# eldenpark/halo2-pse

Measured on AMD Instinct MI355X. Metric: bn254_msm_g1_adds_per_sec, higher is better.
Workload: dtype u32x8 (256-bit Montgomery integers)

## Files before the change

### halo2-pse_amd/csrc/msm.hip

```cpp
#include <hip/hip_ext.h>
#include <string.h>

#include <atomic>
#include <condition_variable>
#include <thread>
#include <vector>

#include "ecq.h"
#include "engine.h"
#include "host64.h"

namespace h2 {

#define MSM_MAX_C1 1024u
#define MSM_MAX_L 12u
#define MSM_STAGE 16384u
#define MSM_COUNT_TILE 4096u

struct MsmPlan {
    uint32_t c;
    uint32_t W;
    uint32_t q;
    uint32_t cb;
    uint32_t NB;
    uint32_t shared;
    uint32_t heavy_t;
    uint32_t chunk;
};

template <class F>
__device__ __forceinline__ void for_each_digit(const Fe& s, uint32_t c, uint32_t q, uint32_t W, F&& f) {
    uint64_t buf = 0;
    uint32_t nb = 0, w = 0, carry = 0;
    uint32_t width = q ? c : c - 1;
    auto emit = [&]() {
        uint32_t d = ((uint32_t)buf & ((1u << width) - 1)) + carry;
        uint32_t neg = 0;
        carry = 0;
        if (d > (1u << (width - 1))) {
            d = (1u << width) - d;
            neg = 1;
            carry = 1;
        }
        if (d) f(w, d - 1, neg);
        w++;
        buf >>= width;
        nb = nb > width ? nb - width : 0;
        width = w < q ? c : c - 1;
    };
#pragma unroll
    for (int limb = 0; limb < 8; limb++) {
        buf |= (uint64_t)s.l[limb] << nb;
        nb += 32;
        while (nb >= width && w < W) emit();
    }
    while (w < W) emit();
}

struct L1Args {
    const Fe* scalars_one;
    const Fe* const* list;
    uint32_t n, c, q, W, cb, L, C1;
    uint32_t shared, stride;
    uint32_t tile;
    uint16_t* tile_hist;
    const uint32_t* tile_off;
    uint2* tmp;
    uint32_t* tmp_e;
    uint16_t* tmp_k;
    const Affine* chk_bases;
    const Affine* chk_samples;
    uint32_t* chk_flag;
    size_t chk_n, chk_total;
};

__device__ __forceinline__ Fe fr_to_canonical(const Fe& x) {
    Fu c32 = fu_zero();
    c32.l[0] = 32;
    return fu_mul_canon<FrU>(fu_slice(x), c32);
}

#define MSM_TCHUNK 64u
#ifndef MSM_SCATTER_XG
#define MSM_SCATTER_XG 4u
#endif

__global__ void __launch_bounds__(256) msm_l1_count_kernel(L1Args a) {
    __shared__ uint32_t lh[MSM_MAX_C1];
    if (a.chk_flag && blockIdx.x == 0 && blockIdx.y == 0 && threadIdx.x < 4 * H2_PIN_SAMPLES) {
        const uint32_t k = threadIdx.x >> 2, part = threadIdx.x & 3;
// ... 94 lines not shown
        for_each_digit(sc, a.c, a.q, a.W, [&](uint32_t w, uint32_t slot, uint32_t neg) {
            const uint32_t gb = ((set0 + (a.shared ? 0u : w)) << a.cb) | slot;
            const uint32_t pos = atomicAdd(&cur[gb >> a.L], 1u);
            stage[pos] = make_uint2((a.shared ? w * a.stride + i : i) | (neg << 31), gb);
        });
    }
    __syncthreads();
    for (uint32_t pos = threadIdx.x; pos < total; pos += 1024) {
        const uint2 e = stage[pos];
        const uint32_t at = pos + delta[e.y >> a.L];
        if (SPLIT) {
            a.tmp_e[at] = e.x;
            a.tmp_k[at] = (uint16_t)(e.y & ((1u << a.L) - 1));
        } else {
            a.tmp[at] = e;
        }
    }
}

__global__ void __launch_bounds__(1024) msm_l1_scan_kernel(uint32_t* __restrict__ chunk_sum, uint32_t n_chunks, uint32_t C1,
                                                           uint32_t* __restrict__ bin_total, uint32_t* __restrict__ zero, uint32_t zero_words) {
    __shared__ uint32_t part_sum[16][64];
    if (blockIdx.x == 0)
        for (uint32_t i = threadIdx.x; i < zero_words; i += 1024) zero[i] = 0;
    const uint32_t lb = threadIdx.x & 63, p = threadIdx.x >> 6, b = blockIdx.x * 64 + lb;
    const uint32_t per = (n_chunks + 15) / 16, c0 = p * per, c1 = c0 + per < n_chunks ? c0 + per : n_chunks;
    uint32_t sum = 0;
    if (b < C1)
        for (uint32_t ch = c0; ch < c1; ch++) sum += chunk_sum[(size_t)ch * C1 + b];
    part_sum[p][lb] = sum;
    __syncthreads();
    uint32_t acc = 0, all = 0;
#pragma unroll
    for (uint32_t q = 0; q < 16; q++) {
        const uint32_t v = part_sum[q][lb];
        if (q < p) acc += v;
        all += v;
    }
    if (b < C1) {
        for (uint32_t ch = c0; ch < c1; ch++) {
            const uint32_t v = chunk_sum[(size_t)ch * C1 + b];
            chunk_sum[(size_t)ch * C1 + b] = acc;
            acc += v;
        }
        if (p == 0) bin_total[b] = all;
    }
}

__global__ void __launch_bounds__(256) msm_l1_offsets_kernel(const uint16_t* __restrict__ tile_hist, uint32_t n_tiles, uint32_t C1,
                                                             const uint32_t* __restrict__ chunk_sum, const uint32_t* __restrict__ bin_total,
                                                             uint32_t* __restrict__ coarse_start, uint32_t* __restrict__ tile_off) {
    __shared__ uint32_t cs[MSM_MAX_C1], ps[4];
    const uint32_t per = (C1 + 255) / 256;
    uint32_t total;
    uint32_t run = block_scan_base<256>(bin_total, C1, per, ps, &total);
    for (uint32_t j = 0; j < per; j++) {
        const uint32_t k = threadIdx.x * per + j;
        if (k < C1) {
            cs[k] = run;
            run += bin_total[k];
        }
    }
    __syncthreads();
    const uint32_t b = blockIdx.y * 256 + threadIdx.x;
    if (b >= C1) return;
    if (blockIdx.x == 0) {
        coarse_start[b] = cs[b];
        if (b == 0) coarse_start[C1] = total;
    }
    const uint32_t t0 = blockIdx.x * MSM_TCHUNK, t1 = t0 + MSM_TCHUNK < n_tiles ? t0 + MSM_TCHUNK : n_tiles;
    uint32_t running = cs[b] + chunk_sum[(size_t)blockIdx.x * C1 + b];
#pragma unroll 8
    for (uint32_t t = t0; t < t1; t++) {
        tile_off[(size_t)t * C1 + b] = running;
        running += tile_hist[(size_t)t * C1 + b];
    }
}

__device__ __forceinline__ uint32_t size_class(uint32_t cnt, uint32_t bin_shift) {
    uint32_t b = cnt >> bin_shift;
    return 255u - (b < 255u ? b : 255u);
}

template <bool SPLIT>
__global__ void __launch_bounds__(1024) msm_l2_kernel(const uint2* __restrict__ tmp, const uint32_t* __restrict__ tmp_e, const uint16_t* __restrict__ tmp_k,
                                                      const uint32_t* __restrict__ coarse_start, uint32_t L,
                                                      uint32_t bin_shift, uint32_t* __restrict__ vals, uint32_t* __restrict__ start,
                                                      uint32_t* __restrict__ counts, uint32_t* __restrict__ perm, uint32_t* __restrict__ class_hist) {
    constexpr uint32_t NBMAX = 1u << MSM_MAX_L, EPT = MSM_STAGE / 1024;
    __shared__ uint32_t sval[MSM_STAGE];
    __shared__ uint16_t skey[MSM_STAGE];
    __shared__ uint32_t gpos[NBMAX];
    __shared__ uint32_t tcur[NBMAX];
    __shared__ uint32_t tdelta[NBMAX];
    __shared__ uint32_t ps[16], cls[256];
    const uint32_t nb = 1u << L, t = threadIdx.x, per = (nb + 1023) / 1024;
    const uint32_t cs = coarse_start[blockIdx.x], ce = coarse_start[blockIdx.x + 1];
    const bool single = ce - cs <= MSM_STAGE;
    auto load_tile = [&](uint2 (&e)[EPT], uint32_t first, uint32_t tile_n) {
#pragma unroll
        for (uint32_t j = 0; j < EPT; j++) {
            const uint32_t idx = t + j * 1024;
            if (idx < tile_n) e[j] = SPLIT ? make_uint2(tmp_e[first + idx], tmp_k[first + idx]) : tmp[first + idx];
        }
    };
    auto count_tile = [&](const uint2 (&e)[EPT], uint32_t tile_n) {
#pragma unroll
        for (uint32_t j = 0; j < EPT; j++)
            if (t + j * 1024 < tile_n) atomicAdd(&tcur[e[j].y & (nb - 1)], 1u);
    };
    uint2 e[EPT], e_next[EPT];
    const uint32_t first_n = ce - cs < MSM_STAGE ? ce - cs : MSM_STAGE;
    load_tile(e, cs, first_n);
    for (uint32_t k = t; k < nb; k += 1024) tcur[k] = 0;
    if (t < 256) cls[t] = 0;
    __syncthreads();
    if (single) {
        count_tile(e, first_n);
    } else {
        uint32_t idx = cs + t;
        for (; idx + 7 * 1024 < ce; idx += 8 * 1024) {
            uint32_t key[8];
#pragma unroll
            for (uint32_t j = 0; j < 8; j++) key[j] = SPLIT ? (uint32_t)tmp_k[idx + j * 1024] : tmp[idx + j * 1024].y;
#pragma unroll
            for (uint32_t j = 0; j < 8; j++) atomicAdd(&tcur[key[j] & (nb - 1)], 1u);
        }
        for (; idx < ce; idx += 1024) atomicAdd(&tcur[(SPLIT ? (uint32_t)tmp_k[idx] : tmp[idx].y) & (nb - 1)], 1u);
    }
    __syncthreads();
    uint32_t total;
    uint32_t run = block_scan_base<1024>(tcur, nb, per, ps, &total);
    const uint32_t gb0 = blockIdx.x << L;
    for (uint32_t j = 0; j < per; j++) {
        const uint32_t k = t * per + j;
        if (k < nb) {
            const uint32_t cnt = tcur[k];
            gpos[k] = cs + run;
            start[gb0 + k] = cs + run;
            counts[gb0 + k] = cnt;
            atomicAdd(&cls[size_class(cnt, bin_shift)], 1u);
            run += cnt;
        }
    }
    __syncthreads();
    if (class_hist) {
        if (t < 256 && cls[t]) atomicAdd(&class_hist[t], cls[t]);
    } else {
        uint32_t dummy;
        const uint32_t c0 = block_scan_base<1024>(cls, 256, 1, ps, &dummy);
        if (t < 256) tdelta[t] = c0;
        __syncthreads();
        for (uint32_t j = 0; j < per; j++) {
            const uint32_t k = t * per + j;
            if (k < nb) perm[gb0 + atomicAdd(&tdelta[size_class(tcur[k], bin_shift)], 1u)] = gb0 + k;
        }
        __syncthreads();
    }
    for (uint32_t base = cs; base < ce; base += MSM_STAGE) {
        const uint32_t tile_n = ce - base < MSM_STAGE ? ce - base : MSM_STAGE;
        const uint32_t next = base + MSM_STAGE;
        const uint32_t next_n = next < ce ? (ce - next < MSM_STAGE ? ce - next : MSM_STAGE) : 0;
        if (next_n) load_tile(e_next, next, next_n);
        if (!single) {
            for (uint32_t k = t; k < nb; k += 1024) tcur[k] = 0;
            __syncthreads();
            count_tile(e, tile_n);
            __syncthreads();
        }
        run = block_scan_base<1024>(tcur, nb, per, ps, &total);
        for (uint32_t j = 0; j < per; j++) {
            const uint32_t k = t * per + j;
            if (k < nb) {
                const uint32_t cnt = tcur[k];
                tdelta[k] = gpos[k] - run;
                gpos[k] += cnt;
                tcur[k] = run;
                run += cnt;
            }
        }
        __syncthreads();
#pragma unroll
        for (uint32_t j = 0; j < EPT; j++) {
            const uint32_t idx = t + j * 1024;
            if (idx < tile_n) {
                const uint32_t k = e[j].y & (nb - 1);
                const uint32_t pos = atomicAdd(&tcur[k], 1u);
                sval[pos] = e[j].x;
                skey[pos] = (uint16_t)k;
            }
        }
        __syncthreads();
        for (uint32_t pos = t; pos < tile_n; pos += 1024) vals[pos + tdelta[skey[pos]]] = sval[pos];
        __syncthreads();
#pragma unroll
        for (uint32_t j = 0; j < EPT; j++) e[j] = e_next[j];
    }
}

#define MSM_BS_PER 4u
struct HeavyBucket {
    uint32_t bucket, first_chunk, n_chunks, arrived;
};
struct HeavyChunk {
    uint32_t begin, end, owner;
};

__global__ void __launch_bounds__(1024) msm_bucket_scatter_kernel(const uint32_t* __restrict__ counts, const uint32_t* __restrict__ start, uint32_t n_buckets,
                                                                  uint32_t bin_shift, uint32_t heavy_t, uint32_t chunk, uint32_t* __restrict__ hist,
                                                                  uint32_t* __restrict__ perm, uint32_t* __restrict__ heavy_counts,
                                                                  HeavyBucket* __restrict__ heavy_buckets, HeavyChunk* __restrict__ heavy_chunks) {
    __shared__ uint32_t scan[256], lh[256], lbase[256], ps[16];
    const uint32_t t = threadIdx.x;
    for (uint32_t j = 0; j < MSM_BS_PER; j++) {
        const uint32_t b = (blockIdx.x * 1024 + t) * MSM_BS_PER + j;
        const uint32_t cnt = b < n_buckets ? counts[b] : 0;
        if (cnt > heavy_t) {
            const uint32_t s0 = start[b], e0 = s0 + cnt, nch = (cnt + chunk - 1) / chunk;
            const uint32_t slot = atomicAdd(&heavy_counts[1], nch);
            const uint32_t hb = atomicAdd(&heavy_counts[0], 1u);
            const HeavyBucket h = {b, slot, nch, 0};
            heavy_buckets[hb] = h;
            for (uint32_t q = 0; q < nch; q++) {
                const HeavyChunk ch = {s0 + q * chunk, (s0 + (q + 1) * chunk < e0) ? s0 + (q + 1) * chunk : e0, hb};
                heavy_chunks[slot + q] = ch;
            }
        }
    }
    if (!perm) return;
    if (t < 256) lh[t] = 0;
    uint32_t total;
    const uint32_t excl = block_scan_base<1024>(hist, 256, 1, ps, &total);
    if (t < 256) scan[t] = excl;
    __syncthreads();
    uint32_t cls[MSM_BS_PER], rank[MSM_BS_PER];
    const uint32_t b0 = (blockIdx.x * 1024 + t) * MSM_BS_PER;
#pragma unroll
    for (uint32_t j = 0; j < MSM_BS_PER; j++) {
        cls[j] = 0;
        rank[j] = 0;
        if (b0 + j < n_buckets) {
            cls[j] = size_class(counts[b0 + j], bin_shift);
            rank[j] = atomicAdd(&lh[cls[j]], 1u);
        }
    }
    __syncthreads();
    if (t < 256 && lh[t]) lbase[t] = atomicAdd(&hist[256 + t], lh[t]);
    __syncthreads();
#pragma unroll
    for (uint32_t j = 0; j < MSM_BS_PER; j++)
        if (b0 + j < n_buckets) perm[scan[cls[j]] + lbase[cls[j]] + rank[j]] = b0 + j;
}

__device__ __noinline__ void msm_heavy_role(const Affine* __restrict__ bases, const uint32_t* __restrict__ vals, const uint32_t* __restrict__ heavy_counts,
                                            HeavyBucket* __restrict__ heavy_buckets, const HeavyChunk* __restrict__ heavy_chunks,
                                            XYZZu* __restrict__ chunk_sums, uint32_t split_log, uint32_t cont, XYZZu* __restrict__ parts, uint32_t hgrid,
                                            XYZZu* sh);

#ifdef H2_ACCUM_TIMELINE
__device__ unsigned long long g_accum_tl[6 * 16384];
#endif
__global__ void __launch_bounds__(256, 4) msm_accum_kernel(const Affine* __restrict__ bases, const uint32_t* __restrict__ vals,
                                                        const uint32_t* __restrict__ start, const uint32_t* __restrict__ counts,
                                                        const uint32_t* __restrict__ perm, uint32_t n_buckets, uint32_t split_log, uint32_t heavy_t,
                                                        uint32_t cont, XYZZu* __restrict__ parts, uint32_t hgrid, const uint32_t* __restrict__ heavy_counts,
                                                        HeavyBucket* __restrict__ heavy_buckets, const HeavyChunk* __restrict__ heavy_chunks,
                                                        XYZZu* __restrict__ chunk_sums) {
    __shared__ __align__(16) unsigned char lds_raw[256 * sizeof(XYZZu)];
    if (blockIdx.x < hgrid) {
        msm_heavy_role(bases, vals, heavy_counts, heavy_buckets, heavy_chunks, chunk_sums, split_log, cont, parts, hgrid, reinterpret_cast<XYZZu*>(lds_raw));
        return;
    }
    uint32_t t = (blockIdx.x - hgrid) * blockDim.x + threadIdx.x;
    if ((t >> split_log) >= n_buckets) return;
    const uint32_t S = 1u << split_log, sub = t & (S - 1);
    const uint32_t b = perm[t >> split_log];
    uint32_t s = start[b], e = s + counts[b];
#ifdef H2_ACCUM_TIMELINE
    const unsigned long long tl0 = wall_clock64(), tc0 = clock64();
// ... 319 lines not shown
        }
    }
    if (role == 0) sh[quad] = acc;
    __syncthreads();
    for (uint32_t stride = G >> 1; stride >= 1; stride >>= 1) {
        if (g < stride) {
            XYZZu x = sh[quad];
            xyzzu_add_q(x, sh[quad + stride], role);
            if (role == 0) sh[quad] = x;
        }
        __syncthreads();
    }
    if (live && g == 0 && role == 0) J.out[task] = sh[quad];
}

__global__ void __launch_bounds__(64) msm_final_quad_kernel(FinalArgs args, uint32_t n_groups, XYZZu* __restrict__ partials, uint32_t* __restrict__ done,
                                                            XYZZ* __restrict__ set_sums) {
    __shared__ XYZZu sh[16];
    __shared__ uint32_t is_last;
    const uint32_t set = blockIdx.x / n_groups, group = blockIdx.x - set * n_groups;
    const uint32_t quad = threadIdx.x >> 2, role = threadIdx.x & 3;
    uint32_t e = group * 16 + quad;
    const XYZZu* base = nullptr;
    uint32_t stride = 0, o = 0, k = 0, nbits = 0;
    bool found = false;
#pragma unroll
    for (uint32_t i = 0; i < 4; i++) {
        if (i < args.n_arr && !found) {
            if (e < args.arr[i].len) {
                found = true;
                base = args.arr[i].base;
                stride = args.arr[i].stride;
                o = args.arr[i].o;
                k = args.arr[i].k;
                nbits = args.arr[i].nbits;
            } else {
                e -= args.arr[i].len;
            }
        }
    }
    XYZZu x = xyzzu_identity();
    if (found) {
        const uint32_t wgt = (e + o) << k;
        if (wgt) x = xyzzu_mul_small_q(base[(size_t)set * stride + e], wgt, nbits, role);
    }
    if (role == 0) sh[quad] = x;
    __syncthreads();
    for (uint32_t st = 8; st >= 1; st >>= 1) {
        if (quad < st) {
            XYZZu a = sh[quad];
            xyzzu_add_q(a, sh[quad + st], role);
            if (role == 0) sh[quad] = a;
        }
        __syncthreads();
    }
    if (n_groups == 1) {
        if (threadIdx.x == 0) set_sums[set] = xyzzu_to_ext(sh[0]);
        return;
    }
    if (threadIdx.x == 0) {
        partials[blockIdx.x] = sh[0];
        __threadfence();
        is_last = atomicAdd(&done[set], 1u) == n_groups - 1;
    }
    __syncthreads();
    if (!is_last) return;
    __builtin_amdgcn_fence(__ATOMIC_ACQUIRE, "agent");
    x = xyzzu_identity();
    if (quad < n_groups) x = partials[(size_t)set * n_groups + quad];
    if (role == 0) sh[quad] = x;
    __syncthreads();
    for (uint32_t st = 8; st >= 1; st >>= 1) {
        if (quad < st) {
            XYZZu a = sh[quad];
            xyzzu_add_q(a, sh[quad + st], role);
            if (role == 0) sh[quad] = a;
        }
        __syncthreads();
    }
    if (threadIdx.x == 0) set_sums[set] = xyzzu_to_ext(sh[0]);
}

#define MSM_PLANES_MAX 32
#define MSM_PLANE_SETS_MAX 4
struct PlaneJob {
    const XYZZu* base;
    uint32_t log_len;
    uint32_t o;
    uint32_t n_planes;
    uint32_t wgs;
    uint32_t first_plane;
    uint32_t first_block;
};
struct PlaneArgs {
    PlaneJob job[2];
    uint32_t blocks_per_set, planes_per_set;
};

__global__ void __launch_bounds__(256) msm_planes_kernel(PlaneArgs args, XYZZu* __restrict__ partials, uint32_t* __restrict__ done,
                                                         XYZZ* __restrict__ plane_sums) {
    __shared__ XYZZu sh[64];
    __shared__ uint32_t is_last;
    const uint32_t set = blockIdx.x / args.blocks_per_set, b = blockIdx.x - set * args.blocks_per_set;
    const PlaneJob& J = args.job[b >= args.job[1].first_block ? 1 : 0];
    const uint32_t pb = b - J.first_block, plane = pb / J.wgs, part = pb - plane * J.wgs;
    const XYZZu* X = J.base + ((size_t)set << J.log_len);
    const uint32_t quad = threadIdx.x >> 2, role = threadIdx.x & 3;
    const bool top = plane == J.log_len;
    const uint32_t count = top ? 1u : 1u << (J.log_len - 1);
    auto elem = [&](uint32_t t) -> XYZZu {
        if (t >= count) return xyzzu_identity();
        const uint32_t v = top ? (1u << J.log_len) : ((t >> plane) << (plane + 1)) | (1u << plane) | (t & ((1u << plane) - 1));
        return X[v - J.o];
    };
    const uint32_t t0 = part * 128 + 2 * quad;
    const XYZZu x = xyzzu_sum_q(elem(t0), elem(t0 + 1), role);
    if (role == 0) sh[quad] = x;
    __syncthreads();
    for (uint32_t st = 32; st >= 1; st >>= 1) {
        if (quad < st) {
            const XYZZu a = xyzzu_sum_q(sh[quad], sh[quad + st], role);
            if (role == 0) sh[quad] = a;
        }
        __syncthreads();
    }
    const uint32_t out = set * args.planes_per_set + J.first_plane + plane;
    if (J.wgs == 1) {
        if (threadIdx.x == 0) plane_sums[out] = xyzzu_to_ext(sh[0]);
        return;
    }
    if (threadIdx.x == 0) {
        partials[(size_t)out * 16 + part] = sh[0];
        __threadfence();
        is_last = atomicAdd(&done[out], 1u) == J.wgs - 1;
    }
    __syncthreads();
    if (!is_last) return;
    __builtin_amdgcn_fence(__ATOMIC_ACQUIRE, "agent");
    XYZZu y = xyzzu_identity();
    if (quad < J.wgs) y = partials[(size_t)out * 16 + quad];
    if (role == 0 && quad < 16) sh[quad] = y;
    __syncthreads();
    for (uint32_t st = 8; st >= 1; st >>= 1) {
        if (quad < st) {
            const XYZZu a = xyzzu_sum_q(sh[quad], sh[quad + st], role);
            if (role == 0) sh[quad] = a;
        }
        __syncthreads();
    }
    if (threadIdx.x == 0) plane_sums[out] = xyzzu_to_ext(sh[0]);
}

__global__ void __launch_bounds__(256) msm_table_step_kernel(const Affine* __restrict__ prev, XYZZ* __restrict__ out, uint32_t n, uint32_t c) {
    const uint32_t i = blockIdx.x * blockDim.x + threadIdx.x;
    if (i >= n) return;
    const Affine p = prev[i];
    if (affine_is_identity(p)) {
        out[i] = xyzz_identity();
        return;
    }
    XYZZu q = xyzzu_double_affine<FqUA>(fu_from_ext(p.x), fu_from_ext(p.y));
    for (uint32_t k = 1; k < c; k++) q = xyzzu_double(q);
    out[i] = xyzzu_to_ext(q);
}

static uint32_t g_window_override = 0;
static size_t g_heavy_div = 32768;
static size_t g_bin_entries = 8192;
static bool g_split_records = true;
void msm_set_split_records(bool on) { g_split_records = on; }
static uint64_t g_rowcol_lanes = 65536;
static bool g_rowcol_asm = true, g_rowcol_qtree = true;
void msm_set_rowcol(uint64_t lanes, uint32_t flavour) {
    g_rowcol_lanes = lanes ? lanes : 65536;
    g_rowcol_asm = flavour & 1;
    g_rowcol_qtree = flavour & 2;
}
static bool g_split_buckets = true;
void msm_set_split_buckets(bool on) { g_split_buckets = on; }
static bool g_quad_tail = true;
void msm_set_quad_tail(bool on) { g_quad_tail = on; }
static bool g_global_order = true;
void msm_set_bucket_order(int local) { g_global_order = local == 0; }
void msm_set_bin_entries(size_t d) { g_bin_entries = d ? d : 8192; }
void msm_set_heavy_div(size_t d) { g_heavy_div = d ? d : 32768; }
static size_t g_max_chunk = (size_t)1 << 26;
void msm_set_max_chunk(size_t m) { g_max_chunk = m ? m : ((size_t)1 << 26); }
static uint32_t g_reserved_cus = 0;
void msm_set_reserved_cus(uint32_t k) { g_reserved_cus = k; }
uint32_t msm_get_reserved_cus() { return g_reserved_cus; }
void msm_set_window(uint32_t c) { g_window_override = c; }

static uint32_t floor_log2(size_t n) {
    uint32_t lg = 0;
    while (((size_t)1 << (lg + 1)) <= n) lg++;
    return lg;
}

static uint32_t plain_window(size_t n, bool fused) {
    if (g_window_override) return g_window_override;
    const uint32_t lg = floor_log2(n);
    if (fused && lg >= 13 && lg <= 18) return lg <= 13 ? 10 : lg <= 16 ? 12 : lg == 17 ? 13 : 14;
    if (lg <= 8) return 7;
    if (lg <= 12) return 10;
    if (lg <= 14) return 13;
    if (lg <= 17) return 15;
    return 17;
}

static uint32_t normalise_window(uint32_t c) {
    if (c < 2) c = 2;
    if (c > 22) c = 22;
    const uint32_t W = (255 + c - 1) / c;
    return (255 + W - 1) / W;
}

uint32_t msm_table_window(size_t n) {
    if (g_window_override) return normalise_window(g_window_override);
    const uint32_t lg = floor_log2(n);
    uint32_t c = lg <= 12 ? 13 : lg <= 17 ? 17 : lg <= 21 ? 20 : 22;
    return normalise_window(c);
}

static MsmPlan make_plan(size_t n, bool fused, const MsmTable* tab, uint32_t force_c = 0) {
    MsmPlan p;
    uint32_t c = tab ? tab->c : force_c ? force_c : plain_window(n, fused);
// ... 123 lines not shown
    L->o_perm = carve((size_t)K * 4);
    L->o_buckets = carve((size_t)K * sizeof(XYZZu));
    L->o_parts = L->split_log ? carve(((size_t)K << L->split_log) * sizeof(XYZZu)) : L->o_buckets;
    L->o_RA = carve(((size_t)ns << L->rb) * sizeof(XYZZu));
    L->o_CA = carve(((size_t)ns << L->s) * sizeof(XYZZu));
    L->o_RR = carve(((size_t)ns << (L->rb - L->s2)) * sizeof(XYZZu));
    L->o_RC = carve(((size_t)ns << L->s2) * sizeof(XYZZu));
    L->o_CR = carve(((size_t)ns << (L->s - L->s3)) * sizeof(XYZZu));
    L->o_CC = carve(((size_t)ns << L->s3) * sizeof(XYZZu));
    L->o_sums = carve((size_t)ns * sizeof(XYZZ));
    L->o_partials = carve((size_t)ns * 16 * sizeof(XYZZu));
    L->o_ppart = carve(ns <= MSM_PLANE_SETS_MAX ? (size_t)ns * MSM_PLANES_MAX * 16 * sizeof(XYZZu) : 0);
    L->o_ptrs = carve((size_t)fuse * sizeof(void*));
    L->o_thist = carve((size_t)L->n_tiles * L->C1 * 2);
    L->o_toff = carve((size_t)L->n_tiles * L->C1 * 4);
    L->o_chsum = carve((size_t)L->n_tchunks * L->C1 * 4);
    L->o_tmp = carve(E * 8);
    L->o_vals = carve(E * 4);
    L->o_hb = carve(L->max_heavy * sizeof(HeavyBucket));
    L->o_hc = carve(L->max_chunks * sizeof(HeavyChunk));
    L->o_hs = carve(L->max_chunks * sizeof(XYZZu));
    L->total = off;
    return 0;
}

static int msm_stage_a(Ctx* c, const MsmLayout& L, char* base, const Fe* const* d_scalars_list, const MsmTable* tab, hipStream_t s) {
    const MsmPlan& p = L.p;
    const size_t n = L.n;
    uint32_t* cstart = (uint32_t*)(base + L.o_cstart);
    uint32_t *vals = (uint32_t*)(base + L.o_vals), *start = (uint32_t*)(base + L.o_start);
    uint32_t *counts = (uint32_t*)(base + L.o_counts), *perm = (uint32_t*)(base + L.o_perm);
    int t0 = c->timer_begin("msm_digits", s);
    L1Args a;
    a.scalars_one = d_scalars_list[0];
    a.list = nullptr;
    if (L.fuse > 1) {
        int rc = c->stage_h2d(base + L.o_ptrs, d_scalars_list, L.fuse * sizeof(void*), s);
        if (rc) return rc;
        a.list = (const Fe* const*)(base + L.o_ptrs);
    }
    a.n = (uint32_t)n;
    a.c = p.c;
    a.q = p.q;
    a.W = p.W;
    a.cb = p.cb;
    a.L = L.L;
    a.C1 = L.C1;
    a.shared = p.shared;
    a.stride = tab ? (uint32_t)tab->stride : 0;
    a.tile = L.tile;
    a.tile_hist = (uint16_t*)(base + L.o_thist);
    a.tile_off = (const uint32_t*)(base + L.o_toff);
    a.tmp = (uint2*)(base + L.o_tmp);
    a.chk_bases = c->pin_chk.bases;
    a.chk_samples = c->pin_chk.samples;
    a.chk_flag = c->pin_chk.flag;
    a.chk_n = c->pin_chk.n;
    a.chk_total = c->pin_chk.total;
    c->pin_chk = Ctx::PinCheck();
    uint32_t* chsum = (uint32_t*)(base + L.o_chsum);
    const dim3 tiles(L.tiles_x, L.fuse), chunks(L.n_tchunks, (L.C1 + 255) / 256);
    hipLaunchKernelGGL(msm_l1_count_kernel, tiles, dim3(256), 0, s, a);
    H2_CHECK(hipGetLastError());
    c->timer_end(t0, s);
    int t1 = c->timer_begin("msm_sort", s);
    hipLaunchKernelGGL(msm_l1_chunk_kernel, chunks, dim3(256), 0, s, (const uint16_t*)a.tile_hist, L.n_tiles, L.C1, chsum);
    H2_CHECK(hipGetLastError());
    uint32_t* bin_total = (uint32_t*)(base + L.o_bintot);
    hipLaunchKernelGGL(msm_l1_scan_kernel, dim3((L.C1 + 63) / 64), dim3(1024), 0, s, chsum, L.n_tchunks, L.C1, bin_total,
                       (uint32_t*)(base + L.o_zero), (uint32_t)((L.o_zero_end - L.o_zero) / 4));
    H2_CHECK(hipGetLastError());
    hipLaunchKernelGGL(msm_l1_offsets_kernel, chunks, dim3(256), 0, s, (const uint16_t*)a.tile_hist, L.n_tiles, L.C1, (const uint32_t*)chsum,
                       (const uint32_t*)bin_total, cstart, (uint32_t*)(base + L.o_toff));
    H2_CHECK(hipGetLastError());
    const bool split = g_split_records && L.E / L.C1 > MSM_STAGE;
    a.tmp_e = (uint32_t*)(base + L.o_tmp);
    a.tmp_k = (uint16_t*)(base + L.o_tmp + L.E * 4);
    if (split)
        hipLaunchKernelGGL(msm_l1_scatter_kernel<true>, tiles, dim3(1024), 0, s, a);
    else
        hipLaunchKernelGGL(msm_l1_scatter_kernel<false>, tiles, dim3(1024), 0, s, a);
    H2_CHECK(hipGetLastError());
    uint32_t* hist = (uint32_t*)(base + L.o_hist);
    if (split)
        hipLaunchKernelGGL(msm_l2_kernel<true>, dim3(L.C1), dim3(1024), 0, s, (const uint2*)nullptr, (const uint32_t*)a.tmp_e, (const uint16_t*)a.tmp_k, cstart,
                           L.L, L.bin_shift, vals, start, counts, perm, g_global_order ? hist : (uint32_t*)nullptr);
    else
        hipLaunchKernelGGL(msm_l2_kernel<false>, dim3(L.C1), dim3(1024), 0, s, (const uint2*)(base + L.o_tmp), (const uint32_t*)nullptr,
                           (const uint16_t*)nullptr, cstart, L.L, L.bin_shift, vals, start, counts, perm, g_global_order ? hist : (uint32_t*)nullptr);
    H2_CHECK(hipGetLastError());
    hipLaunchKernelGGL(msm_bucket_scatter_kernel, dim3((L.K + 1024 * MSM_BS_PER - 1) / (1024 * MSM_BS_PER)), dim3(1024), 0, s, (const uint32_t*)counts,
                       (const uint32_t*)start, L.K, L.bin_shift, p.heavy_t, p.chunk, hist, g_global_order ? perm : (uint32_t*)nullptr,
                       (uint32_t*)(base + L.o_hcnt), (HeavyBucket*)(base + L.o_hb), (HeavyChunk*)(base + L.o_hc));
    H2_CHECK(hipGetLastError());
    c->timer_end(t1, s);
    return 0;
}

static int msm_stage_b(Ctx* c, const MsmLayout& L, char* base, const Affine* d_points, hipStream_t s, char* bbase = nullptr, bool cont = false,
                       bool combine = true) {
    const MsmPlan& p = L.p;
    if (!bbase) bbase = base;
    uint32_t* vals = (uint32_t*)(base + L.o_vals);
    uint32_t *start = (uint32_t*)(base + L.o_start), *counts = (uint32_t*)(base + L.o_counts), *perm = (uint32_t*)(base + L.o_perm);
    XYZZu* buckets = (XYZZu*)(bbase + L.o_buckets);
    uint32_t* hcnt = (uint32_t*)(base + L.o_hcnt);
    HeavyBucket* hb = (HeavyBucket*)(base + L.o_hb);
    HeavyChunk* hc = (HeavyChunk*)(base + L.o_hc);
    XYZZu* hs = (XYZZu*)(base + L.o_hs);
    int t2 = c->timer_begin("msm_accum", s);
    hipEvent_t ke0 = nullptr, ke1 = nullptr;
    XYZZu* parts = (XYZZu*)(bbase + L.o_parts);
    const uint32_t lanes = L.K << L.split_log;
    const uint32_t cont_u = cont ? 1u : 0u;
    const uint32_t hgrid = (uint32_t)(L.max_chunks < (size_t)c->sm_count ? L.max_chunks : (size_t)c->sm_count);
    const dim3 agrid(hgrid + (lanes + 255) / 256);
    if (c->timer_kernel("msm_accum", &ke0, &ke1) >= 0)
        hipExtLaunchKernelGGL(msm_accum_kernel, agrid, dim3(256), 0, s, ke0, ke1, 0, d_points, (const uint32_t*)vals, (const uint32_t*)start,
                              (const uint32_t*)counts, (const uint32_t*)perm, L.K, L.split_log, p.heavy_t, cont_u, parts, hgrid, (const uint32_t*)hcnt, hb,
                              (const HeavyChunk*)hc, hs);
    else
        hipLaunchKernelGGL(msm_accum_kernel, agrid, dim3(256), 0, s, d_points, (const uint32_t*)vals, (const uint32_t*)start, (const uint32_t*)counts,
                           (const uint32_t*)perm, L.K, L.split_log, p.heavy_t, cont_u, parts, hgrid, (const uint32_t*)hcnt, hb, (const HeavyChunk*)hc, hs);
    H2_CHECK(hipGetLastError());
    c->timer_end(t2, s);
    if (L.split_log && combine) {
        const uint32_t comb_lanes = L.K << (L.split_log - 1);
        hipLaunchKernelGGL(msm_combine_kernel, dim3((comb_lanes + 255) / 256), dim3(256), 0, s, (const XYZZu*)parts, L.K, L.split_log, buckets);
        H2_CHECK(hipGetLastError());
    }
    return 0;
}

static void rowcol_jobs(RowColArgs* ra, const XYZZu* in, XYZZu* out_rows, XYZZu* out_cols, uint32_t n_arr, uint32_t log_rows, uint32_t log_cols,
                        uint32_t* n_blocks, bool quad = false) {
    const uint64_t elems = (uint64_t)n_arr << (log_rows + log_cols);
    const uint64_t budget = (2 * elems) >> 4 > g_rowcol_lanes ? 2 * g_rowcol_lanes : g_rowcol_lanes;
    uint32_t t_log = 1;
    while (!quad && (2 * elems) >> t_log > budget) t_log++;
    for (uint32_t kind = 0; kind < 2; kind++) {
        RowColJob* j = &ra->job[ra->n_jobs++];
        const uint32_t log_terms = kind ? log_rows : log_cols, log_sums = kind ? log_cols : log_rows;
        uint32_t g_log = log_terms > t_log ? log_terms - t_log : 0;
        const uint32_t g_max = quad ? 4 : 8;
        if (g_log > g_max) g_log = g_max;
        j->in = in;
        j->out = kind ? out_cols : out_rows;
        j->n_arr = n_arr;
        j->log_rows = log_rows;
        j->log_cols = log_cols;
        j->cols_kind = kind;
        j->g_log = g_log;
        j->first_block = *n_blocks;
        const uint64_t tasks = (uint64_t)n_arr << log_sums;
        const uint32_t per_block = (quad ? 16u : 256u) >> g_log;
        *n_blocks += (uint32_t)((tasks + per_block - 1) / per_block);
    }
}

static bool g_plane_tail = true;
void msm_set_plane_tail(bool on) { g_plane_tail = on; }
static bool msm_plane_tail(const Ctx* c, const MsmLayout& L) {
    return g_plane_tail && g_quad_tail && L.levels >= 1 && L.n_sets <= MSM_PLANE_SETS_MAX && L.rb <= 11 && L.s <= 11 && L.rb >= 1 && L.s >= 1 &&
           L.s + 1 + L.rb <= MSM_PLANES_MAX && !c->gather_want;
}
static inline uint32_t msm_planes_per_set(const MsmLayout& L) { return L.rb + L.s + 1; }

static void msm_planes_finish(const MsmLayout& L, const XYZZ* planes, XYZZ* sums) {
    const uint32_t pps = msm_planes_per_set(L);
    for (uint32_t set = 0; set < L.n_sets; set++) {
        const XYZZ* P = planes + (size_t)set * pps;
        h64::P acc = h64::identity();
        for (uint32_t m = L.s + L.rb; m-- > 0;) {
            acc = h64::pdouble(acc);
            if (m >= L.s) h64::padd(acc, h64::from_xyzz(P[L.s + 1 + (m - L.s)]));
            if (m <= L.s) h64::padd(acc, h64::from_xyzz(P[m]));
        }
        sums[set] = h64::to_xyzz(acc);
    }
}

static int msm_stage_c(Ctx* c, const MsmLayout& L, char* base, XYZZ* h_sums, hipStream_t s, XYZZ* h_planes = nullptr) {
    XYZZu* buckets = (XYZZu*)(base + L.o_buckets);
    XYZZu *RA = (XYZZu*)(base + L.o_RA), *CA = (XYZZu*)(base + L.o_CA), *RR = (XYZZu*)(base + L.o_RR), *RC = (XYZZu*)(base + L.o_RC);
    XYZZu *CR = (XYZZu*)(base + L.o_CR), *CC = (XYZZu*)(base + L.o_CC);
    const bool direct = !c->gather_want;
    XYZZ* sums = direct ? h_sums : (XYZZ*)(base + L.o_sums);
    const uint32_t ns = L.n_sets, cb = L.p.cb;
    const bool quad = g_quad_tail && ns <= 64;
    int t4 = c->timer_begin("msm_reduce", s);
    FinalArgs fa;
    memset(&fa, 0, sizeof(fa));
    auto set_arr = [&](uint32_t i, const XYZZu* b, uint32_t log_len, uint32_t o, uint32_t k) {
        fa.arr[i].base = b;
        fa.arr[i].stride = 1u << log_len;
        fa.arr[i].len = 1u << log_len;
        fa.arr[i].o = o;
        fa.arr[i].k = k;
        fa.arr[i].nbits = bits_of(((1u << log_len) - 1 + o) << k);
    };
    if (L.levels == 0) {
        set_arr(0, buckets, cb, 1, 0);
        fa.n_arr = 1;
    } else {
        RowColArgs ra;
        memset(&ra, 0, sizeof(ra));
        uint32_t nblk = 0;
        rowcol_jobs(&ra, buckets, RA, CA, ns, L.rb, L.s, &nblk);
        if (g_rowcol_qtree)
            hipLaunchKernelGGL(msm_rowcol_qtree_kernel<FqUA>, dim3(nblk), dim3(256), 0, s, ra);
        else if (g_rowcol_asm)
            hipLaunchKernelGGL(msm_rowcol_kernel<FqUA>, dim3(nblk), dim3(256), 0, s, ra);
        else
            hipLaunchKernelGGL(msm_rowcol_kernel<FqU>, dim3(nblk), dim3(256), 0, s, ra);
        H2_CHECK(hipGetLastError());
        if (h_planes && msm_plane_tail(c, L)) {
            PlaneArgs pa;
            memset(&pa, 0, sizeof(pa));
            uint32_t blk = 0, pl = 0;
            for (uint32_t k = 0; k < 2; k++) {
                PlaneJob& J = pa.job[k];
                J.base = k ? RA : CA;
                J.log_len = k ? L.rb : L.s;
                J.o = k ? 0 : 1;
                J.n_planes = J.log_len + J.o;
                J.wgs = J.log_len > 7 ? 1u << (J.log_len - 8) : 1;
                J.first_plane = pl;
                J.first_block = blk;
                pl += J.n_planes;
                blk += J.n_planes * J.wgs;
            }
            pa.blocks_per_set = blk;
            pa.planes_per_set = pl;
            hipLaunchKernelGGL(msm_planes_kernel, dim3(ns * blk), dim3(256), 0, s, pa, (XYZZu*)(base + L.o_ppart), (uint32_t*)(base + L.o_fdone), h_planes);
            H2_CHECK(hipGetLastError());
            c->timer_end(t4, s);
            return 0;
        }
        if (L.levels == 1) {
            set_arr(0, RA, L.rb, 0, L.s);
            set_arr(1, CA, L.s, 1, 0);
            fa.n_arr = 2;
        } else {
            memset(&ra, 0, sizeof(ra));
            nblk = 0;
            rowcol_jobs(&ra, RA, RR, RC, ns, L.rb - L.s2, L.s2, &nblk, quad);
            rowcol_jobs(&ra, CA, CR, CC, ns, L.s - L.s3, L.s3, &nblk, quad);
            if (quad)
                hipLaunchKernelGGL(msm_rowcol_quad_kernel, dim3(nblk), dim3(64), 0, s, ra);
            else
                hipLaunchKernelGGL(msm_rowcol_kernel<FqU>, dim3(nblk), dim3(256), 0, s, ra);
            H2_CHECK(hipGetLastError());
            set_arr(0, RR, L.rb - L.s2, 0, L.s + L.s2);
            set_arr(1, RC, L.s2, 0, L.s);
            set_arr(2, CR, L.s - L.s3, 0, L.s3);
            set_arr(3, CC, L.s3, 1, 0);
            fa.n_arr = 4;
        }
    }
    if (quad) {
        uint32_t n_el = 0;
        for (uint32_t i = 0; i < fa.n_arr; i++) n_el += fa.arr[i].len;
        const uint32_t n_groups = (n_el + 15) / 16;
        XYZZu* partials = (XYZZu*)(base + L.o_partials);
        hipLaunchKernelGGL(msm_final_quad_kernel, dim3(ns * n_groups), dim3(64), 0, s, fa, n_groups, partials, (uint32_t*)(base + L.o_fdone), sums);
    } else {
        hipLaunchKernelGGL(msm_final_kernel, dim3(ns), dim3(256), 0, s, fa, sums);
    }
    H2_CHECK(hipGetLastError());
    c->timer_end(t4, s);
    if (!direct) H2_CHECK(hipMemcpyAsync(h_sums, sums, (size_t)ns * sizeof(XYZZ), hipMemcpyDeviceToHost, s));
    if (c->gather_want) {
        const size_t bytes = (size_t)ns * sizeof(XYZZ);
        if (c->gather_off + bytes <= H2_GATHER_OWN && c->gather.p)
            H2_CHECK(hipMemcpyAsync((char*)c->gather.p + c->gather_off, sums, bytes, hipMemcpyDeviceToDevice, s));
        c->gather_off += bytes;
    }
    return 0;
}

static inline uint32_t sets_per_msm(const MsmPlan& p) { return p.shared ? 1 : p.W; }
static inline XYZZ finish_msm(const XYZZ* sums, const MsmPlan& p) { return p.shared ? sums[0] : combine_windows(sums, p); }

static int msm_batch_chunk(Ctx* c, const Fe* const* d_scalars, bool scalars_on_host, const Affine* d_points, const MsmTable* tab, size_t n,
                           size_t count, XYZZ* h_out, hipStream_t s) {
    MsmLayout L;
    int rc = msm_layout(n, &L, 1, tab);
    if (rc) return rc;
    const size_t n_slots = count < 3 ? count : 3;
    for (size_t k = 0; k < n_slots; k++) {
        rc = c->msm_slot[k].ensure(L.total);
        if (rc) return rc;
        if (scalars_on_host) {
            rc = c->msm_scalars[k].ensure(n * sizeof(Fe));
            if (rc) return rc;
        }
    }
    auto scalars_for = [&](size_t j, hipStream_t st, const Fe** out) -> int {
        if (!scalars_on_host) {
            *out = d_scalars[j];
            return 0;
        }
        Fe* dst = (Fe*)c->msm_scalars[j % 3].p;
        H2_CHECK(hipMemcpyAsync(dst, d_scalars[j], n * sizeof(Fe), hipMemcpyHostToDevice, st));
        *out = dst;
        return 0;
    };
    const uint32_t spm = sets_per_msm(L.p);
    rc = c->host_ws.ensure(count * spm * sizeof(XYZZ));
// ... 382 lines not shown
```

### include/halo2hip_debug.h

```cpp
#ifndef HALO2HIP_DEBUG_H
#define HALO2HIP_DEBUG_H
#include "halo2hip.h"

#ifdef __cplusplus
extern "C" {
#endif

int h2hip_debug_set_msm_stream(uint32_t chunks, uint32_t ratio_permille, size_t min_n);
size_t h2hip_debug_msm_stream_ladder(size_t n, uint32_t chunks, uint32_t ratio_permille, int with_bases, size_t* sizes, size_t cap);
int h2hip_debug_set_msm_max_chunk(size_t m);
int h2hip_debug_rccl_gather_selftest(const uint64_t* partials_xyz, size_t count, uint64_t* out_xyz);
int h2hip_debug_set_msm_heavy_div(size_t d);
int h2hip_debug_set_g2l_quad(int on);
int h2hip_debug_set_msm_fuse_limits(size_t entries, size_t max_n);
int h2hip_debug_set_msm_rowcol(uint64_t lanes, int use_asm);
int h2hip_debug_set_msm_split_buckets(int on);
int h2hip_debug_set_msm_plane_tail(int on);
int h2hip_debug_set_msm_quad_tail(int on);
int h2hip_debug_set_msm_bucket_order(int local);
int h2hip_debug_set_msm_split_records(int on);
int h2hip_debug_set_msm_bin_entries(size_t d);
int h2hip_debug_set_reserved_cus(uint32_t k);
int h2hip_debug_set_msm_fuse_small(int on);
int h2hip_debug_set_ntt_smax(uint32_t v);
int h2hip_debug_ntt_plan(uint32_t log_n, size_t count, uint32_t radices[4]);
int h2hip_debug_set_lazy_pin(uint32_t after);
int h2hip_debug_set_ntt_two_pass(uint32_t lo, uint32_t hi);
int h2hip_debug_set_ntt_twiddle_budget(uint64_t bytes);
int h2hip_debug_set_ntt_batch_bytes(uint64_t bytes);
int h2hip_debug_set_ntt_two_pass_batch_wgs(uint64_t v);
int h2hip_debug_set_ntt_full_max_log_m(uint32_t v);
int h2hip_debug_set_ntt_fold_tables(int on);
int h2hip_debug_set_ntt_host_batch(uint64_t run_bytes, uint64_t group_bytes);
int h2hip_debug_set_ntt_two_pass_log_j(int v);
int h2hip_debug_set_evalh_max_local_slots(uint32_t v);
int h2hip_debug_set_evalh_lookup_group_bytes(uint64_t v);
int h2hip_debug_evalh_program_muls(const h2hip_graph* g, uint32_t* n_mul);
int h2hip_debug_set_evalh_codegen(int mode, uint32_t max_ops);
int h2hip_debug_evalh_codegen_source(const h2hip_graph* g, char* buf, size_t cap, size_t* len, int compile, double* seconds, size_t* code_bytes);
int h2hip_debug_evalh_codegen_stats(uint64_t out[5]);
int h2hip_debug_evalh_compile_stats(const h2hip_graph* g, uint32_t* n_ops, uint32_t* n_slots);
int h2hip_debug_set_opening_tile(uint32_t rows_per_thread, uint32_t threads_per_tile);
int h2hip_debug_set_lookup_sort(uint32_t lds_keys);
int h2hip_debug_lookup_sort_stats(uint32_t out[2]);
int h2hip_debug_set_keygen_group(uint64_t group_bytes);

#ifdef __cplusplus
}
#endif
#endif
```

Baseline: 11.19 billion.

## Size level-2 sort tiles to fill LDS and balance planes reduction for small lengths

The level-2 bucket sort kernel is templated on the bucket count so each instantiation sizes its staging tile to fill about 160 KiB of LDS instead of a fixed 16K entries. Larger coarse bins are split into evenly sized tiles. The register double buffer (e_next) is dropped; the next tile is now loaded before the scatter to global memory instead. Separately, the planes reduction derives its workgroup count and reduction depth from the actual plane length, so short planes no longer run empty reduction steps. A debug entry point that reports the layout is added. The risks are lower occupancy from the larger LDS use and less load/compute overlap.

```diff
diff --git a/halo2-pse_amd/csrc/msm.hip b/halo2-pse_amd/csrc/msm.hip
--- a/halo2-pse_amd/csrc/msm.hip
+++ b/halo2-pse_amd/csrc/msm.hip
@@ -6,6 +6,7 @@
 #include <thread>
 #include <vector>
 
+#include "../../include/halo2hip_debug.h"
 #include "ecq.h"
 #include "engine.h"
 #include "host64.h"
@@ -266,21 +267,36 @@
     return 255u - (b < 255u ? b : 255u);
 }
 
-template <bool SPLIT>
+template <uint32_t LB>
+struct L2Plan {
+    static constexpr uint32_t NB = 1u << LB;
+    static constexpr uint32_t FIXED = (16 + 256) * 4;
+    static constexpr uint32_t EPT = (160u * 1024 - FIXED - 3 * 4 * NB) / (6 * 1024);
+    static constexpr uint32_t CAP = EPT * 1024;
+};
+static_assert(L2Plan<9>::CAP == 25600 && L2Plan<10>::CAP == 24576 && L2Plan<11>::CAP == 22528 && L2Plan<12>::CAP == 18432, "level-2 tile table");
+static inline uint32_t msm_l2_cap(uint32_t L) {
+    return L <= 9 ? L2Plan<9>::CAP : L == 10 ? L2Plan<10>::CAP : L == 11 ? L2Plan<11>::CAP : L2Plan<12>::CAP;
+}
+
+template <bool SPLIT, uint32_t LB>
 __global__ void __launch_bounds__(1024) msm_l2_kernel(const uint2* __restrict__ tmp, const uint32_t* __restrict__ tmp_e, const uint16_t* __restrict__ tmp_k,
                                                       const uint32_t* __restrict__ coarse_start, uint32_t L,
                                                       uint32_t bin_shift, uint32_t* __restrict__ vals, uint32_t* __restrict__ start,
                                                       uint32_t* __restrict__ counts, uint32_t* __restrict__ perm, uint32_t* __restrict__ class_hist) {
-    constexpr uint32_t NBMAX = 1u << MSM_MAX_L, EPT = MSM_STAGE / 1024;
-    __shared__ uint32_t sval[MSM_STAGE];
-    __shared__ uint16_t skey[MSM_STAGE];
+    constexpr uint32_t NBMAX = L2Plan<LB>::NB, EPT = L2Plan<LB>::EPT, CAP = L2Plan<LB>::CAP;
+    __shared__ uint32_t sval[CAP];
+    __shared__ uint16_t skey[CAP];
     __shared__ uint32_t gpos[NBMAX];
     __shared__ uint32_t tcur[NBMAX];
     __shared__ uint32_t tdelta[NBMAX];
     __shared__ uint32_t ps[16], cls[256];
     const uint32_t nb = 1u << L, t = threadIdx.x, per = (nb + 1023) / 1024;
     const uint32_t cs = coarse_start[blockIdx.x], ce = coarse_start[blockIdx.x + 1];
-    const bool single = ce - cs <= MSM_STAGE;
+    const uint32_t n = ce - cs;
+    const bool single = n <= CAP;
+    const uint32_t n_tiles = (n + CAP - 1) / CAP;
+    const uint32_t tile = single ? CAP : ((n + n_tiles - 1) / n_tiles + 63) & ~63u;
     auto load_tile = [&](uint2 (&e)[EPT], uint32_t first, uint32_t tile_n) {
 #pragma unroll
         for (uint32_t j = 0; j < EPT; j++) {
@@ -293,8 +309,8 @@
         for (uint32_t j = 0; j < EPT; j++)
             if (t + j * 1024 < tile_n) atomicAdd(&tcur[e[j].y & (nb - 1)], 1u);
     };
-    uint2 e[EPT], e_next[EPT];
-    const uint32_t first_n = ce - cs < MSM_STAGE ? ce - cs : MSM_STAGE;
+    uint2 e[EPT];
+    const uint32_t first_n = n < tile ? n : tile;
     load_tile(e, cs, first_n);
     for (uint32_t k = t; k < nb; k += 1024) tcur[k] = 0;
     if (t < 256) cls[t] = 0;
@@ -341,11 +357,8 @@
         }
         __syncthreads();
     }
-    for (uint32_t base = cs; base < ce; base += MSM_STAGE) {
-        const uint32_t tile_n = ce - base < MSM_STAGE ? ce - base : MSM_STAGE;
-        const uint32_t next = base + MSM_STAGE;
-        const uint32_t next_n = next < ce ? (ce - next < MSM_STAGE ? ce - next : MSM_STAGE) : 0;
-        if (next_n) load_tile(e_next, next, next_n);
+    for (uint32_t base = cs; base < ce; base += tile) {
+        const uint32_t tile_n = ce - base < tile ? ce - base : tile;
         if (!single) {
             for (uint32_t k = t; k < nb; k += 1024) tcur[k] = 0;
             __syncthreads();
@@ -375,10 +388,10 @@
             }
         }
         __syncthreads();
+        const uint32_t next = base + tile;
+        if (next < ce) load_tile(e, next, ce - next < tile ? ce - next : tile);
         for (uint32_t pos = t; pos < tile_n; pos += 1024) vals[pos + tdelta[skey[pos]]] = sval[pos];
         __syncthreads();
-#pragma unroll
-        for (uint32_t j = 0; j < EPT; j++) e[j] = e_next[j];
     }
 }
 
@@ -864,6 +877,7 @@
 }
 
 #define MSM_PLANES_MAX 32
+#define MSM_PLANE_POINTS 128u
 #define MSM_PLANE_SETS_MAX 4
 struct PlaneJob {
     const XYZZu* base;
@@ -895,11 +909,12 @@
         const uint32_t v = top ? (1u << J.log_len) : ((t >> plane) << (plane + 1)) | (1u << plane) | (t & ((1u << plane) - 1));
         return X[v - J.o];
     };
-    const uint32_t t0 = part * 128 + 2 * quad;
-    const XYZZu x = xyzzu_sum_q(elem(t0), elem(t0 + 1), role);
+    const uint32_t m = count < MSM_PLANE_POINTS ? count : MSM_PLANE_POINTS;
+    const uint32_t t0 = part * MSM_PLANE_POINTS + 2 * quad;
+    const XYZZu x = m > 1 ? xyzzu_sum_q(elem(t0), elem(t0 + 1), role) : elem(part * MSM_PLANE_POINTS + quad);
     if (role == 0) sh[quad] = x;
     __syncthreads();
-    for (uint32_t st = 32; st >= 1; st >>= 1) {
+    for (uint32_t st = m >> 2; st >= 1; st >>= 1) {
         if (quad < st) {
             const XYZZu a = xyzzu_sum_q(sh[quad], sh[quad + st], role);
             if (role == 0) sh[quad] = a;
@@ -923,7 +938,7 @@
     if (quad < J.wgs) y = partials[(size_t)out * 16 + quad];
     if (role == 0 && quad < 16) sh[quad] = y;
     __syncthreads();
-    for (uint32_t st = 8; st >= 1; st >>= 1) {
+    for (uint32_t st = J.wgs >> 1; st >= 1; st >>= 1) {
         if (quad < st) {
             const XYZZu a = xyzzu_sum_q(sh[quad], sh[quad + st], role);
             if (role == 0) sh[quad] = a;
@@ -1213,12 +1228,23 @@
         hipLaunchKernelGGL(msm_l1_scatter_kernel<false>, tiles, dim3(1024), 0, s, a);
     H2_CHECK(hipGetLastError());
     uint32_t* hist = (uint32_t*)(base + L.o_hist);
-    if (split)
-        hipLaunchKernelGGL(msm_l2_kernel<true>, dim3(L.C1), dim3(1024), 0, s, (const uint2*)nullptr, (const uint32_t*)a.tmp_e, (const uint16_t*)a.tmp_k, cstart,
-                           L.L, L.bin_shift, vals, start, counts, perm, g_global_order ? hist : (uint32_t*)nullptr);
+    auto launch_l2 = [&](auto plan) {
+        constexpr uint32_t LB = decltype(plan)::value;
+        if (split)
+            hipLaunchKernelGGL((msm_l2_kernel<true, LB>), dim3(L.C1), dim3(1024), 0, s, (const uint2*)nullptr, (const uint32_t*)a.tmp_e, (const uint16_t*)a.tmp_k,
+                               cstart, L.L, L.bin_shift, vals, start, counts, perm, g_global_order ? hist : (uint32_t*)nullptr);
+        else
+            hipLaunchKernelGGL((msm_l2_kernel<false, LB>), dim3(L.C1), dim3(1024), 0, s, (const uint2*)(base + L.o_tmp), (const uint32_t*)nullptr,
+                               (const uint16_t*)nullptr, cstart, L.L, L.bin_shift, vals, start, counts, perm, g_global_order ? hist : (uint32_t*)nullptr);
+    };
+    if (L.L <= 9)
+        launch_l2(std::integral_constant<uint32_t, 9>());
+    else if (L.L == 10)
+        launch_l2(std::integral_constant<uint32_t, 10>());
+    else if (L.L == 11)
+        launch_l2(std::integral_constant<uint32_t, 11>());
     else
-        hipLaunchKernelGGL(msm_l2_kernel<false>, dim3(L.C1), dim3(1024), 0, s, (const uint2*)(base + L.o_tmp), (const uint32_t*)nullptr,
-                           (const uint16_t*)nullptr, cstart, L.L, L.bin_shift, vals, start, counts, perm, g_global_order ? hist : (uint32_t*)nullptr);
+        launch_l2(std::integral_constant<uint32_t, 12>());
     H2_CHECK(hipGetLastError());
     hipLaunchKernelGGL(msm_bucket_scatter_kernel, dim3((L.K + 1024 * MSM_BS_PER - 1) / (1024 * MSM_BS_PER)), dim3(1024), 0, s, (const uint32_t*)counts,
                        (const uint32_t*)start, L.K, L.bin_shift, p.heavy_t, p.chunk, hist, g_global_order ? perm : (uint32_t*)nullptr,
@@ -1291,11 +1317,36 @@
 
 static bool g_plane_tail = true;
 void msm_set_plane_tail(bool on) { g_plane_tail = on; }
-static bool msm_plane_tail(const Ctx* c, const MsmLayout& L) {
+static bool msm_plane_geometry(const MsmLayout& L) {
     return g_plane_tail && g_quad_tail && L.levels >= 1 && L.n_sets <= MSM_PLANE_SETS_MAX && L.rb <= 11 && L.s <= 11 && L.rb >= 1 && L.s >= 1 &&
-           L.s + 1 + L.rb <= MSM_PLANES_MAX && !c->gather_want;
-}
+           L.s + 1 + L.rb <= MSM_PLANES_MAX;
+}
+static bool msm_plane_tail(const Ctx* c, const MsmLayout& L) { return msm_plane_geometry(L) && !c->gather_want; }
 static inline uint32_t msm_planes_per_set(const MsmLayout& L) { return L.rb + L.s + 1; }
+static inline uint32_t msm_plane_wgs(uint32_t log_len) {
+    const uint32_t count = 1u << (log_len - 1);
+    return count > MSM_PLANE_POINTS ? count / MSM_PLANE_POINTS : 1;
+}
+
+}
+extern "C" int h2hip_debug_msm_layout(size_t n, uint32_t fuse, uint32_t fixed_c, uint32_t out[8]) {
+    using namespace h2;
+    if (!out || !n) {
+        set_error("msm_layout: null output or no pairs");
+        return H2HIP_EINVAL;
+    }
+    MsmTable tab;
+    tab.c = normalise_window(fixed_c);
+    tab.W = (255 + tab.c - 1) / tab.c;
+    tab.stride = n;
+    MsmLayout L;
+    if (msm_layout(n, &L, fuse ? fuse : 1, fixed_c ? &tab : nullptr)) return H2HIP_EINVAL;
+    const bool planes = msm_plane_geometry(L);
+    const uint32_t v[8] = {L.p.c, L.p.W, L.L, L.C1, msm_l2_cap(L.L), planes ? 1u : 0u, planes ? msm_plane_wgs(L.s) : 0u, planes ? msm_plane_wgs(L.rb) : 0u};
+    memcpy(out, v, sizeof(v));
+    return 0;
+}
+namespace h2 {
 
 static void msm_planes_finish(const MsmLayout& L, const XYZZ* planes, XYZZ* sums) {
     const uint32_t pps = msm_planes_per_set(L);
@@ -1355,7 +1406,7 @@
                 J.log_len = k ? L.rb : L.s;
                 J.o = k ? 0 : 1;
                 J.n_planes = J.log_len + J.o;
-                J.wgs = J.log_len > 7 ? 1u << (J.log_len - 8) : 1;
+                J.wgs = msm_plane_wgs(J.log_len);
                 J.first_plane = pl;
                 J.first_block = blk;
                 pl += J.n_planes;
diff --git a/include/halo2hip_debug.h b/include/halo2hip_debug.h
--- a/include/halo2hip_debug.h
+++ b/include/halo2hip_debug.h
@@ -17,6 +17,7 @@
 int h2hip_debug_set_msm_split_buckets(int on);
 int h2hip_debug_set_msm_plane_tail(int on);
 int h2hip_debug_set_msm_quad_tail(int on);
+int h2hip_debug_msm_layout(size_t n, uint32_t fuse, uint32_t fixed_c, uint32_t out[8]);
 int h2hip_debug_set_msm_bucket_order(int local);
 int h2hip_debug_set_msm_split_records(int on);
 int h2hip_debug_set_msm_bin_entries(size_t d);
```

New measurement: 11.25 billion (median of 6 runs). No clear change (+0.6%).
